# zz9tf/multimodal-fusion

Measured on AMD Instinct MI355X. Metric: similarity-pairs/sec (NxN cosine+top-k), higher is better.
Workload: dtype f16 MFMA scan + f32 exact re-rank; 1 GPU; N=262144 d=512 single-modality cosine + top-5, self excluded, f32 features, unit-norm Gaussian rows; rows_per_rank=262144, parallelism=single GPU, driver=single, scan_kernel=scan_b16x<f16> (v_mfma_f32_16x16x32_f16), col_splits=1, scan_grid=2048, fallback_rows=0, overflow_rows=0, query_order=False, near_duplicate_rows_estimate=0

## Files before the change

### multimodal-fusion_amd/csrc/mmf_api.hip

```cpp
#include <stdarg.h>
#include <string.h>

#include <algorithm>
#include <map>
#include <mutex>
#include <optional>
#include <utility>
#include <vector>

#include "mmf_host.h"

namespace mmf {

static thread_local char g_err[512] = "";

void set_error(const char* fmt, ...) {
  va_list ap;
  va_start(ap, fmt);
  vsnprintf(g_err, sizeof(g_err), fmt, ap);
  va_end(ap);
}

struct WsEntry { char* base = nullptr; size_t cap = 0; WsKept kept; };
static std::mutex g_ws_mu;
// ... 253 lines not shown
  int32_t* fail_rows = nullptr; uint32_t *fail_count = nullptr, *cand_total = nullptr;
  uint32_t h_fail4[4] = {0, 0, 0, 0};
  std::vector<uint32_t> h_tot;
  static size_t bytes(int64_t n) { return ws_bytes(n, 4) + ws_bytes(4, 4) + ws_bytes(256, 4); }
  void carve(Workspace& ws, int64_t n) { fail_rows = ws.take<int32_t>(n); fail_count = ws.take<uint32_t>(4); cand_total = ws.take<uint32_t>(256); }
  int zero(hipStream_t s) const {
    MMF_HIP(hipMemsetAsync(fail_count, 0, 16, s)); MMF_HIP(hipMemsetAsync(cand_total, 0, 1024, s));
    return MMF_OK;
  }
  int read(bool totals, hipStream_t s) {
    MMF_HIP(hipMemcpyAsync(h_fail4, fail_count, 16, hipMemcpyDeviceToHost, s));
    h_tot.assign(totals ? 256 : 0, 0);
    if (totals) MMF_HIP(hipMemcpyAsync(h_tot.data(), cand_total, 1024, hipMemcpyDeviceToHost, s));
    MMF_HIP(hipStreamSynchronize(s));
    return MMF_OK;
  }
};

static void symmetric_live_mode(bool* live, bool* forward) {
  const char* e = getenv("MMF_SYMMETRIC_LIVE");
  const int v = e ? atoi(e) : 1;
  *live = (v == 1 || v == 2);
  *forward = (v == 0 || v == 2);
}
static bool symmetric_prune_mode() {
  const char* e = getenv("MMF_SYMMETRIC_PRUNE");
  return !e || atoi(e) != 0;
}
static bool wide_sink_mode() {
  const char* e = getenv("MMF_WIDE_SINK");
  return !e || atoi(e) != 0;
}
static constexpr int64_t kSymMinRows = 131072;
static bool symmetric_scan_wanted(int64_t n, int dp, int bcap, int metric, int forced_splits, bool same_ids, int* G) {
  if (!same_ids || dp != 512 || bcap != scan_bf16_cap(1, 512) || forced_splits != 0) return false;
  if (metric != MMF_DOT && metric != MMF_COSINE) return false;
  const int64_t nb = (n + 255) / 256;
  if (nb * 256 * 1024 >= (int64_t(1) << 32)) return false;
  const char* e = getenv("MMF_SYMMETRIC");
  const int mode = e ? atoi(e) : -1;
  if (mode == 0 || (mode < 0 && n < kSymMinRows)) return false;
  int g = sym_default_group(nb);
  if (const char* ge = getenv("MMF_SYMMETRIC_G")) { const int v = atoi(ge); if (v >= 1 && v <= 65536) g = v; }
  *G = g;
  return true;
}
// ... 152 lines not shown
  int64_t n, m; int kk, cap, bcap, splits, lists, fb_splits; int64_t FB;
  CandLists L;
  ExactLists XL;
  FlagBlock flags;
  char* scan_scratch = nullptr;
  char* order_scratch = nullptr;
  int order_mode = MMF_QUERY_ORDER_OFF; bool order_try = false;
  char* qo_scratch = nullptr; uint16_t* qo_Z = nullptr; float *qo_zn = nullptr, *qo_rn = nullptr, *qo_un = nullptr;
  int64_t n_pad_q() const { return (n + 255) / 256 * 256; }
  int set_query_order(int mode) {
    if (mode < MMF_QUERY_ORDER_AUTO || mode > MMF_QUERY_ORDER_ON) { set_error("simtopk: bad query_order %d", mode); return MMF_E_INVALID; }
    order_mode = mode;
    order_try = !wide && (mode == MMF_QUERY_ORDER_ON || (mode == MMF_QUERY_ORDER_AUTO && n >= 32768 && m >= 32768));
    return MMF_OK;
  }

  bool sym_try = false; int sym_G = 32; int lists_alloc = 0;
  SymBuffers sym;
  WsKept sym_kept; WsKept* sym_keep = nullptr;
  uint32_t* sym_cnt = nullptr; uint2* sym_ent = nullptr;
  int64_t sym_grid() const { return sym_schedule_grid((n + 255) / 256, sym_G); }
  void set_symmetric(int G) {
    sym_try = true; sym_G = G;
    if (lists_alloc < 4) lists_alloc = 4;
  }
  CandLists view(bool symmetric) const {
    CandLists v = L;
    v.lists = symmetric ? 4 : lists;
    if (v.lists <= 2) { v.keys = nullptr; v.margin = nullptr; }
    v.spill_stacks = spill_stacks_for(v.lists);
    if (symmetric) { v.sym_cnt = sym_cnt; v.sym_ent = sym_ent; v.sym_cap = kSymCap; }
    return v;
  }

  int dp, panels;
  bool wide = false;
  int panel_splits[16]; int max_splits = 1;
  int64_t n_seed;
  int32_t* seed = nullptr;
  int64_t seed_stripes() const { return wide ? 3 : 2; }
  static constexpr int64_t kRowsExactMax = 48;
  int64_t rows_exact_cap = 0;
  float* row_keys = nullptr;
  bool leave_floors = false; int out_stride = 0;
  float* floor_key_out = nullptr; uint32_t* floor_id_out = nullptr;
  int64_t failed_rows = 0;
  FastTail(int64_t n_, int64_t m_, int kk_, int forced_splits, int dp_, int panels_ = 1, int64_t m_panel_min = -1,
           int64_t m_panel_max = -1)
      : n(n_), m(m_), kk(kk_), cap(scan_f32_cap(kk_)), dp(dp_), panels(panels_) {
    wide = dp > 1024;
    bcap = wide ? scan_b16w_cap(kk) : scan_bf16_cap(kk, dp);
// ... 78 lines not shown
      if (order_mode == MMF_QUERY_ORDER_ON || near_rows >= 8 * (int64_t)query_order_pivots()) {
        MMF_TRY(launch_query_order_apply(fo.q.Z, fo.q.zn, fo.q.rn, fo.q.un, n, n_pad_q(), fo.dp, fo.f16, qo_scratch, qo_Z, qo_zn, qo_rn, qo_un, &fo.perm, s));
        fo.q.Z = qo_Z; fo.q.zn = qo_zn; fo.q.rn = qo_rn; fo.q.un = qo_un;
      }
      MMF_TRY(t_order.stop(s));
    }
    const bool symmetric = sym_try && !fo.perm && fo.n_panels == 0;
    const CandLists L = view(symmetric);
    MMF_HIP(hipMemsetAsync(L.overflow, 0, (size_t)n * 4, s));
    MMF_TRY(flags.zero(s));
    EventTimer t_scan, t_sel, t_fb;
    EventTimer t_panel[16];
    int grid = 0;
    MMF_HIP(hipMemsetAsync(seed, 0x80, (size_t)n_seed * 4 * seed_stripes(), s));
    MMF_HIP(hipMemsetAsync(L.spill_cnt, 0, (size_t)n * 4, s));
    MMF_TRY(t_scan.start(profile, s));
    ScanB16Panel pn;
    pn.seed = seed; pn.seed_stride = n_seed;
    pn.share = (splits > 1 || fo.n_panels > 1) ? 1 : 0;
    ScanB16Problem sp(fo.q, fo.c, n, m, fo.m_pad_tiles, fo.dp, r.d, fo.f16, r.metric, kk);
    if (symmetric) {
      bool live, forward;
      symmetric_live_mode(&live, &forward);
      const WsKept tables{sym.sched, (n + 255) / 256, sym_G, forward ? 1 : 0};
      MMF_TRY(launch_scan_b16_sym(sp, SymLaunch{sym_G, live, forward, symmetric_prune_mode(), !(sym_kept == tables)}, L, scan_scratch, sym,
                                  pn, s, &grid));
      if (sym_keep) *sym_keep = tables;
    } else if (fo.n_panels == 0) {
      if (wide) {
        CandLists Lw = L;
        if (!wide_sink_mode()) { Lw.spill_cnt = nullptr; Lw.spill_ids = nullptr; Lw.spill_cap = 0; Lw.spill_stacks = 0; }
        pn.sunk = seed + 2 * n_seed;
        MMF_TRY(launch_scan_b16w(sp, splits, Lw, pn, s, &grid));
      }
      else MMF_TRY(launch_scan_b16(sp, splits, L, scan_scratch, pn, s, &grid));
    } else {
      int list_base = 0;
      for (int p = 0; p < fo.n_panels; ++p) {
        const mmf_panel& P = fo.panels[p];
        if (P.ready_event) MMF_HIP(hipStreamWaitEvent(s, static_cast<hipEvent_t>(P.ready_event), 0));
        MMF_TRY(t_panel[p].start(profile, s));
        pn.list_base = list_base;
        list_base += 2 * panel_splits[p];
        pn.seg_len = (uint32_t)P.seg_len; pn.seg_stride = (uint32_t)P.seg_stride; pn.id_off = (uint32_t)P.id_base;
        sp.ZC = P.Z; sp.cb = P.cb; sp.m = P.m; sp.m_pad = P.m_pad;
        MMF_TRY(launch_scan_b16(sp, panel_splits[p], L, scan_scratch, pn, s, &grid));
        MMF_TRY(t_panel[p].stop(s));
      }
    }
    MMF_TRY(launch_scan_b16_audit(pn, L.overflow, n, s));
    if (const char* e = getenv("MMF_DEBUG_FLAG_ROWS")) {
      const int64_t f = atoll(e);
      if (f > 0) MMF_HIP(hipMemsetAsync(L.overflow, 1, (size_t)(f < n ? f : n) * 4, s));
    }
    MMF_TRY(t_scan.stop(s));
    if (symmetric && getenv("MMF_SYMMETRIC_DEBUG")) {
      MMF_HIP(hipStreamSynchronize(s));
      std::vector<uint32_t> hc((size_t)n), hl((size_t)sym_grid() * 8);
      uint32_t none = 0;
      MMF_HIP(hipMemcpy(hc.data(), sym_cnt, hc.size() * 4, hipMemcpyDeviceToHost));
      MMF_HIP(hipMemcpy(hl.data(), sym.log_cnt, hl.size() * 4, hipMemcpyDeviceToHost));
      MMF_HIP(hipMemcpy(&none, sym.none_cnt, 4, hipMemcpyDeviceToHost));
      unsigned long long tot = 0, logged = 0; uint32_t mx = 0, lmx = 0;
      for (uint32_t v : hc) { tot += v; if (v > mx) mx = v; }
      for (uint32_t v : hl) { logged += v; if (v > lmx) lmx = v; }
      bool live, forward;
      symmetric_live_mode(&live, &forward);
      fprintf(stderr, "[mmf symmetric] G %d grid %lld %s %s: rows without a threshold %u, received entries %llu (%.1f per row, largest %u of %d), fullest wave log %u of %d, logged entries %llu (%.1f per row, filing %s)\n",
              sym_G, (long long)sym_grid(), live ? "live" : "frozen", forward ? "ahead" : "back", none, tot, (double)tot / (double)n, mx,
              kSymCap, lmx, kSymLogPerWave, logged, (double)logged / (double)n, symmetric_prune_mode() ? "pruned" : "complete");
    }
    if (select_wait_event) MMF_HIP(hipStreamWaitEvent(s, static_cast<hipEvent_t>(select_wait_event), 0));

    SelectProblem q = r.select();
    q.rx = fo.rx; q.cy = fo.cy; q.perm = fo.perm;
    q.fail_rows = flags.fail_rows; q.fail_count = flags.fail_count; q.cand_total = r.stats ? flags.cand_total : nullptr;
    q.two_pass = true;
    q.order_scratch = getenv("MMF_SELECT_UNORDERED") ? nullptr : order_scratch;
    q.out_stride = out_stride;
    if (leave_floors) { q.floor_key_out = floor_key_out; q.floor_id_out = floor_id_out; }
    MMF_TRY(t_sel.start(profile, s));
    MMF_TRY(launch_select(q, L, s));
    MMF_TRY(t_sel.stop(s));

    MMF_TRY(flags.read(r.stats != nullptr, s));
    const uint32_t* h_fail4 = flags.h_fail4;
    const uint32_t h_fail = h_fail4[0];
    failed_rows = h_fail;
    if (h_fail > 0 && getenv("MMF_DEBUG_PRINT_FLAGGED")) {
      const uint32_t nshow = h_fail < 8 ? h_fail : 8;
      int32_t rows[8];
      MMF_HIP(hipMemcpy(rows, flags.fail_rows, nshow * sizeof(int32_t), hipMemcpyDeviceToHost));
      for (uint32_t i = 0; i < nshow; ++i) {
// ... 650 lines not shown
  if (!one) { MMF_TRY(t[0].stop(s)); MMF_TRY(t[1].start(r.profile, s)); }
  std::vector<uint32_t> h_tot(stats ? 256 : 0);
  MMF_TRY(ex.run(ws, B, one ? t : nullptr, stats ? &h_tot : nullptr));
  if (!one) MMF_TRY(t[1].stop(s));
  fill_stats(stats, MMF_PREC_EXACT, ex.splits(ex.pieces[0]), ex.grid, t[0].ms(), t[1].ms(), t[2].ms(), 0.f, 0, 0, 0, h_tot);
  return MMF_OK;
}

}

using namespace mmf;

extern "C" {

int mmf_version(void) { return MMF_ABI_VERSION; }
int mmf_debug_query_order(int32_t* perm_host, int64_t n) { return query_order_last(perm_host, n); }
int64_t mmf_debug_symmetric_schedule(int64_t row_blocks, int group, int launch, int32_t* table_host, int64_t capacity) {
  if (row_blocks < 1 || group < 1 || launch < 0 || launch > 1) { set_error("debug_symmetric_schedule: bad argument"); return MMF_E_INVALID; }
  const int64_t grid = sym_schedule_grid(row_blocks, group);
  if (table_host) {
    if (capacity < grid) { set_error("debug_symmetric_schedule: table of %lld entries needed", (long long)grid); return MMF_E_INVALID; }
    bool live, forward;
    symmetric_live_mode(&live, &forward);
    sym_schedule_table(row_blocks, group, launch, table_host, forward);
  }
  return grid;
}
const char* mmf_last_error(void) { return g_err; }

int mmf_release_workspaces(void) {
  std::lock_guard<std::mutex> lk(g_ws_mu);
  query_order_forget();
  for (auto& slot : g_ws) {
    for (auto& kv : slot) {
      if (kv.second.base) {
        int prev = -1;
        (void)hipGetDevice(&prev);
        (void)hipSetDevice(kv.first.first);
        (void)hipDeviceSynchronize();
        (void)hipFree(kv.second.base);
        if (prev >= 0) (void)hipSetDevice(prev);
      }
    }
    slot.clear();
  }
  for (auto& kv : g_stage) {
    int prev = -1;
// ... 2825 lines not shown
```

### multimodal-fusion_amd/csrc/mmf_host.h

```cpp
#pragma once
#include <hip/hip_runtime.h>
#include <functional>
#include <optional>
#include <stdint.h>
#include <stdio.h>

#include <string>
#include <vector>

#include "../../include/mmf_hg.h"
#include "../../include/mmf_hg_topk.h"
#include "../../include/mmf_hg_topk16.h"
#include "../../include/ext/mmf_hg_topk16_seg.h"
#include "../../include/ext/mmf_hg_topk_xy.h"
#include "../../include/ext/mmf_hg_seg_exact.h"
#include "../../include/ext/mmf_hg_topk_anyk.h"
#include "../../include/ext/mmf_hg_kmeans_ragged.h"
#include "../../include/ext/mmf_hg_cross_seg.h"
#include "../../include/ext/mmf_hg_cross_seg16.h"
#include "../../include/ext/mmf_hg_cross_segw.h"
#include "../../include/ext/mmf_hg_fast_anyk.h"
#include "../../include/ext/mmf_hg_wide_anyk.h"
#include "../../include/ext/mmf_hg_seg_anyk.h"
#include "../../include/ext/mmf_hg_cross_seg_anyk.h"
// ... 11 lines not shown
      mmf::set_error("%s failed: %s (%s:%d)", #call, hipGetErrorString(_e), __FILE__, __LINE__); \
      return MMF_E_HIP;                                                                    \
    }                                                                                      \
  } while (0)

#define MMF_LAUNCH_CHECK()                                                                 \
  do {                                                                                     \
    hipError_t _e = hipGetLastError();                                                     \
    if (_e != hipSuccess) {                                                                \
      mmf::set_error("kernel launch failed: %s (%s:%d)", hipGetErrorString(_e), __FILE__, __LINE__); \
      return MMF_E_HIP;                                                                    \
    }                                                                                      \
  } while (0)

#define MMF_TRY(expr)            \
  do {                           \
    int _rc = (expr);            \
    if (_rc != MMF_OK) return _rc; \
  } while (0)

struct WsKept {
  const void* where = nullptr;
  int64_t row_blocks = 0;
  int group = 0, forward = 0;
  bool operator==(const WsKept& o) const { return where == o.where && row_blocks == o.row_blocks && group == o.group && forward == o.forward; }
};

struct Workspace {
  char* base = nullptr;
  size_t cap = 0;
  size_t off = 0;
  WsKept kept;
  WsKept* keep = nullptr;
  void reset() { off = 0; }
  template <typename T>
  T* take(size_t count) {
    size_t bytes = (count * sizeof(T) + 255) & ~size_t(255);
    T* p = reinterpret_cast<T*>(base + off);
    off += bytes;
    return p;
  }
};
inline size_t ws_bytes(size_t count, size_t elem) { return (count * elem + 255) & ~size_t(255); }

int upload_table(hipStream_t s, void* dst, const void* src_host, size_t bytes);

struct DeviceGuard {
  int prev = -1;
// ... 48 lines not shown


int launch_row_scalars(const void* X, int64_t n, int64_t d, int dtype, int metric, float* out,
                       uint32_t* max_n, hipStream_t s);

struct CandLists {
  uint32_t* cnt;
  uint32_t* ids;
  uint32_t* overflow;
  int lists;
  int cap;
  float* keys = nullptr;
  float* margin = nullptr;
  int slot_ulp = 16;
  uint32_t* spill_cnt = nullptr;
  uint32_t* spill_ids = nullptr;
  int spill_cap = 0;
  int spill_stacks = 0;
  uint32_t* sym_cnt = nullptr;
  uint2* sym_ent = nullptr;
  int sym_cap = 0;
};

int64_t sym_schedule_grid(int64_t nb, int G);
void sym_schedule_table(int64_t nb, int G, int launch, int32_t* out, bool forward = false);
int sym_default_group(int64_t nb);
constexpr int kSymCap = 512;
constexpr int kSymLogPerWave = 4096;
struct SymBuffers {
  float* thr = nullptr;
  uint32_t* log = nullptr;
  uint32_t* log_cnt = nullptr;
  int32_t* sched = nullptr;
  uint32_t* none_cnt = nullptr;
  static size_t bytes(int64_t n_pad, int64_t grid) {
    return ws_bytes(n_pad, 4) + ws_bytes((size_t)grid * 8 * kSymLogPerWave * 4, 4) + ws_bytes((size_t)grid * 8, 4) +
           ws_bytes((size_t)grid * 16, 4) + ws_bytes(4, 4);
  }
  void carve(Workspace& ws, int64_t n_pad, int64_t grid) {
    thr = ws.take<float>(n_pad); log = ws.take<uint32_t>((size_t)grid * 8 * kSymLogPerWave * 4);
    log_cnt = ws.take<uint32_t>((size_t)grid * 8); sched = ws.take<int32_t>((size_t)grid * 16); none_cnt = ws.take<uint32_t>(4);
  }
};

struct ScanB16Panel {
  int list_base = 0;
  uint32_t seg_len = 0, seg_stride = 0, id_off = 0;
  int32_t* seed = nullptr;
// ... 103 lines not shown
};
struct PrepRows { const void* X; int64_t n, d; int dtype, metric; const float* scal; const uint32_t* max_n; };
int launch_prep_half(const PrepRows& r, const HalfImage& out, int dp, bool f16, hipStream_t s);
int launch_prep_half_gather(const PrepRows& r, const int32_t* gather, int64_t n_pos, const HalfImage& out, int dp, bool f16, hipStream_t s);

struct ScanB16Problem {
  const void* ZQ; const float *q_zn, *q_rn, *q_un;
  const void* ZC; const float* cb; const uint32_t* maxima;
  int64_t n_rows, m, m_pad;
  int dp; int64_t d; bool f16; int metric, kk;
  ScanB16Problem(const HalfImage& q, const HalfImage& c, int64_t n_rows_, int64_t m_, int64_t m_pad_, int dp_, int64_t d_, bool f16_,
                 int metric_, int kk_)
      : ZQ(q.Z), q_zn(q.zn), q_rn(q.rn), q_un(q.un), ZC(c.Z), cb(c.cb), maxima(c.maxima), n_rows(n_rows_), m(m_), m_pad(m_pad_),
        dp(dp_), d(d_), f16(f16_), metric(metric_), kk(kk_) {}
};
int launch_scan_b16(const ScanB16Problem& p, int col_splits, const CandLists& L, void* scratch, const ScanB16Panel& pn, hipStream_t s,
                    int* grid_out);
int launch_scan_b16_audit(const ScanB16Panel& pn, uint32_t* overflow, int64_t n_rows, hipStream_t s);
int launch_scan_b16_ceil(const ScanB16Problem& p, int col_splits, const CandLists& L, void* scratch, const ScanB16Panel& pn, const float* ceil,
                         hipStream_t s, int* grid_out);
int launch_scan_b16_ceilings(const ScanB16Problem& p, int cap, const float* floor_key, const float* rx, const uint32_t* max_n, float lambda,
                             int64_t n_pad, float* ceil, hipStream_t s);
size_t scan_b16_sym_scratch_bytes(int64_t n_rows, int G);
struct SymLaunch { int G; bool live, forward, prune, tables; };
int launch_scan_b16_sym(const ScanB16Problem& p, const SymLaunch& y, const CandLists& L, void* scratch, const SymBuffers& sb,
                        const ScanB16Panel& pn, hipStream_t s, int* grid_out);
size_t scan_b16_scratch_bytes(int64_t n_rows, int col_splits, int dp, int cap);
int scan_bf16_slot_ulp(int cap);
int scan_b16_queries_per_block(int dp);
size_t scan_b16_seg_scratch_bytes(int64_t grid, int dp, int cap);
int launch_scan_b16_seg(const ScanB16Problem& p, const int32_t* sched, int64_t grid, const CandLists& L, void* scratch,
                        const ScanB16Panel& pn, hipStream_t s);
int launch_scan_b16_seg_ceil(const ScanB16Problem& p, const int32_t* sched, int64_t grid, const CandLists& L, void* scratch,
                             const ScanB16Panel& pn, const float* ceil, hipStream_t s);
int launch_scan_b16_ceilings_gather(const ScanB16Problem& p, int cap, const int32_t* gather, int64_t n_pos, const float* floor_key, const float* rx,
                                    const uint32_t* max_n, float lambda, int64_t nq_pad, float* ceil, hipStream_t s);
int launch_scan_b16_xseg(const ScanB16Problem& p, const int32_t* sched, int64_t grid, const uint32_t* bounds, const CandLists& L,
                         void* scratch, const ScanB16Panel& pn, hipStream_t s);
int launch_scan_b16_xseg_ceil(const ScanB16Problem& p, const int32_t* sched, int64_t grid, const uint32_t* bounds, const CandLists& L,
                              void* scratch, const ScanB16Panel& pn, const float* ceil, hipStream_t s);

struct AnykStage { const int64_t* idx; const float* val; const float* key; int64_t n; int depth; int64_t col_offset; };
int launch_anyk_count(const AnykStage& st, const int32_t* fail_rows, const uint32_t* fail_count, const float* floor_key, const uint32_t* floor_id,
                      int32_t* certified, uint32_t* hist, hipStream_t s);
int launch_anyk_emit(const AnykStage& st, const int32_t* certified, int t, int done, int out_stride, int64_t* out_idx, float* out_val,
                     float* floor_key, uint32_t* floor_id, int32_t* rescan_rows, uint32_t* rescan_count, hipStream_t s);
int launch_anyk_iota(int32_t* rows, int64_t n, hipStream_t s);
// ... 162 lines not shown
```

### multimodal-fusion_amd/csrc/mmf_scan_bf16.hip

```cpp
#include <stdlib.h>

#include <type_traits>

#include "mmf_dev.h"
#include "mmf_host.h"

namespace mmf {

constexpr int B_CT = 32;
#ifndef MMF_B_CAP
#define MMF_B_CAP 15
#endif
constexpr int B_CAP = MMF_B_CAP;
constexpr int B_CAP_BIG = 16;
constexpr int B_CAP_WIDE = 32;

typedef __bf16 bf16x8_t __attribute__((ext_vector_type(8)));
typedef _Float16 f16x8_t __attribute__((ext_vector_type(8)));
typedef uint32_t u32x4 __attribute__((ext_vector_type(4)));

struct PrepArgs {
  const void* X; int64_t n; int64_t d; int dtype; int metric;
  const float* scal;
  const uint32_t* max_n;
// ... 137 lines not shown
  int share;
  int kk;
  int metric;
  int d;
  int debug;
  unsigned long long* dbg;
  uint32_t* lids;
  uint32_t* cand_cnt; uint32_t* cand_ids; uint32_t* overflow;
  float* cand_keys;
  float* margin_out;
  uint32_t* spill_cnt; uint32_t* spill_ids; int spill_cap;
  int spill_stacks;
  const int32_t* sched;
  float* sym_thr;
  int sym_live;
  uint32_t* sym_log;
  uint32_t* sym_log_cnt;
  int sym_log_cap;
  const uint32_t* xbounds;
  const float* ceil;
};

enum { SEG_QPOS = 0, SEG_ROW0 = 1, SEG_NQ = 2, SEG_T0 = 3, SEG_T1 = 4, SEG_IDOFF = 5, SEG_ENTRY = 8 };
enum { SYM_RB = 0, SYM_B1 = 1, SYM_N1 = 2, SYM_B2 = 3, SYM_N2 = 4 };
enum { XSEG_SLOT = 5, XSEG_W0 = 6, XSEG_W1 = 7 };

__device__ __forceinline__ int32_t seed_enc(float f) {
  const int32_t b = __float_as_int(f);
  return b >= 0 ? b : (b ^ 0x7fffffff);
}
constexpr int32_t kSeedNone = (int32_t)0x80808080;

__device__ __forceinline__ float scan_margin(int metric, int d, int dp, int cap, float zn, float rn, float un, const uint32_t* maxima) {
  const float ZB = __uint_as_float(maxima[0]), RB = __uint_as_float(maxima[1]);
  const float UB = __uint_as_float(maxima[2]), CB = __uint_as_float(maxima[3]);
  const float g_acc = (float)(dp + 8) * 5.9604645e-8f;
  const float g_chain = (float)(d + 2) * 5.9604645e-8f;
  const float slot_eps = (cap <= 16) ? 1.9073486e-6f : 3.8146973e-6f;
  const float e1 = rn * ZB + un * RB + (g_acc + slot_eps) * (zn * ZB + CB);
  float e2;
  if (metric == MMF_DOT) e2 = g_chain * un * UB;
  else if (metric == MMF_COSINE) e2 = (g_chain + 4.7683716e-7f) * un * UB * 1.01f;
  else e2 = g_chain * un * UB + 2.3841858e-7f * (un * un + UB * UB);
  return 2.0f * (e1 + e2) * 1.001f + 1e-30f;
}

__device__ __forceinline__ void glds4(const void* gptr, const void* lptr) {
// ... 38 lines not shown

  const int tid = threadIdx.x;
  const int lane = tid & 63;
  const int wave = __builtin_amdgcn_readfirstlane(tid >> 6);
  const int khalf = SPLITK ? wave / NQW : 0;
  const int qw = SPLITK ? wave % NQW : wave;
  const bool owner = khalf == 0;
  const int half = lane >> 5;
  const int g = lane >> 4;
  const int c16 = lane & 15;
  const int ownb = g & 1;
  const int c = c16 + 16 * ownb;

  int64_t rb;
  int split;
  int64_t t_begin, t_end, row0 = 0;
  int nq = 0;
  uint32_t id_off = a.id_off;
  int sym_n1 = 0, sym_skip = 0;
  int xw0 = 0, xw1 = 0;
  if constexpr (SYM != 0) {
    const int32_t* e = a.sched + (size_t)blockIdx.x * SEG_ENTRY;
    if (e[SYM_RB] < 0) return;
    rb = e[SYM_RB]; split = 0;
    t_begin = e[SYM_B1]; t_end = t_begin + e[SYM_N1] + e[SYM_N2];
    sym_n1 = e[SYM_N1]; sym_skip = e[SYM_B2] - (e[SYM_B1] + e[SYM_N1]);
  } else if constexpr (SEG) {
    const int32_t* e = a.sched + (size_t)blockIdx.x * SEG_ENTRY;
    rb = e[SEG_QPOS] / QT; row0 = e[SEG_ROW0]; nq = e[SEG_NQ];
    t_begin = e[SEG_T0]; t_end = e[SEG_T1];
    if constexpr (XSEG) {
      id_off = 0u; split = e[XSEG_SLOT];
      xw0 = e[XSEG_W0] - e[SEG_T0]; xw1 = e[XSEG_W1] - e[SEG_T0];
    } else {
      id_off = (uint32_t)e[SEG_IDOFF];
      split = 0;
    }
  } else {
    const int CS = a.conc_splits;
    const int64_t round = blockIdx.x / a.blocks_per_round;
    const int64_t j = blockIdx.x - round * a.blocks_per_round;
    const int64_t q = j >> 3;
    const int x = (int)(j & 7);
    split = (int)round * CS + x % CS;
    rb = q * (8 / CS) + x / CS;
    if (rb >= a.row_blocks) return;
    t_begin = (int64_t)split * a.tiles_per_split;
// ... 208 lines not shown
        const uint32_t j0 = id_base + (uint32_t)tt * B_CT + 4u * (uint32_t)g;
#pragma unroll
        for (int cb = 0; cb < 2; ++cb) {
#pragma unroll
          for (int jj = 0; jj < 4; ++jj) {
            const uint32_t j = j0 + 16u * cb + jj;
            if ((uint32_t)(j - b0.x) < b0.y) x.t[cb][0][jj] = kNegInf;
            if ((uint32_t)(j - b1.x) < b1.y) x.t[cb][1][jj] = kNegInf;
          }
        }
      }
    }
  };
  float thr_q0, thr_q1;
  auto refresh_thr = [&]() {
    const float mine = list.thr;
    const float theirs = __shfl_xor(mine, 16);
    thr_q0 = ownb ? theirs : mine;
    thr_q1 = ownb ? mine : theirs;
  };
  refresh_thr();

  constexpr bool SYMCNT = SYM != 0 && MMF_SYM_COUNT != 0;
  auto filter = [&](const Acc& acc, int tt, float m0, float m1) {
    if (__builtin_expect(!(DBG && (a.debug & 1)) && !(SYM != 0 && (MMF_SYM_ABLATE_Q & SYM) != 0) && __any((m0 >= thr_q0) || (m1 >= thr_q1)), 0)) {
      uint32_t id0 = id_base + (uint32_t)tt * B_CT;
      if constexpr (SYM != 0) id0 += (tt >= sym_n1) ? (uint32_t)(sym_skip * B_CT) : 0u;
      f32x16 v;
#pragma unroll
      for (int cb = 0; cb < 2; ++cb) {
#pragma unroll
        for (int j = 0; j < 4; ++j) {
          const float mine = ownb ? acc.t[cb][1][j] : acc.t[cb][0][j];
          const float give = ownb ? acc.t[cb][0][j] : acc.t[cb][1][j];
          v[4 * cb + j] = mine;
          v[8 + 4 * cb + j] = __shfl_xor(give, 16);
        }
      }
      if constexpr (CEIL) {
        float ce;
        if constexpr (XSEG) {
          const int ln = (int)__builtin_amdgcn_mbcnt_hi(~0u, __builtin_amdgcn_mbcnt_lo(~0u, 0u));
          ce = (a.ceil + (q0 + 32 * qw))[(ln & 15) + (ln & 16)];
        } else ce = a.ceil[qop];
#pragma unroll
        for (int r = 0; r < 16; ++r) v[r] = (v[r] > ce) ? kNegInf : v[r];
      }
// ... 188 lines not shown
  if (a.spill_stacks && a.spill_cnt) {
    const uint32_t mine = qvalid ? list.sink.cpos : 0u;
    const uint32_t theirs = (uint32_t)__shfl_xor((int)mine, 32);
    if (mine + theirs > (uint32_t)a.spill_cap) list.lost = kFltMax;
    if (qvalid && half == 0 && (mine | theirs)) a.spill_cnt[qpos] = mine | (theirs << 16);
  }
  sync_seed();
  if constexpr (SYM == 2) {
    if (MMF_SYM_ABLATE == 3) sym_wcnt = 0;
    if (lane == 0) a.sym_log_cnt[(size_t)blockIdx.x * NW + wave] = sym_wcnt < (uint32_t)a.sym_log_cap ? sym_wcnt : (uint32_t)a.sym_log_cap;
  }
  if (qvalid) {
    const int64_t lbase = qpos * a.lists_total + a.list_base + 2 * split + half;
    a.cand_cnt[lbase] = (uint32_t)list.cnt;
    for (int e = 0; e < list.cnt; ++e) {
      uint32_t id = list.id_of(e);
      if (a.seg_len) id = (id / a.seg_len) * a.seg_stride + id % a.seg_len;
      a.cand_ids[lbase * CAP + e] = id + id_off;
      if (a.cand_keys) a.cand_keys[lbase * CAP + e] = list.keys[e * NTL];
    }
    if (a.cand_keys && half == 0) a.margin_out[qpos] = margin;
    if (list.lost > kNegInf) atomicMax(a.lost + qpos, seed_enc(list.lost) + SlotList<CAP, NTL>::SLOTS);
  }
}

__global__ void audit_kernel(const int32_t* seed, const int32_t* lost, uint32_t* overflow, int64_t n) {
  const int64_t i = (int64_t)blockIdx.x * blockDim.x + threadIdx.x;
  if (i >= n) return;
  const int32_t l = lost[i];
  if (l > kSeedNone && l >= seed[i]) overflow[i] = 1u;
}

struct CeilArgs {
  const float* floor_key; const float* rx;
  const float *q_zn, *q_rn, *q_un; const uint32_t* maxima; const uint32_t* max_n;
  int64_t n, n_pad; int metric, d, dp, cap; float lambda;
  float* ceil;
  const int32_t* gather;
};
template <bool GATHER>
__global__ void ceil_kernel(CeilArgs a) {
  const int64_t i = (int64_t)blockIdx.x * blockDim.x + threadIdx.x;
  if (i >= a.n_pad) return;
  if (i >= a.n) { a.ceil[i] = __builtin_huge_valf(); return; }
  int64_t row = i;
  if constexpr (GATHER) {
// ... 284 lines not shown
    return launch_b16_t<64, 8, 1, B_CAP, true, true, 0, true, true>(a, f16, grid, s);
  }
  set_error("scan_b16_xseg_ceil: no kernel for padded dim %d with %d-entry lists (full-depth passes only)", dp, cap);
  return MMF_E_INTERNAL;
}

int launch_scan_b16_xseg_ceil(const ScanB16Problem& p, const int32_t* sched, int64_t grid, const uint32_t* bounds, const CandLists& L,
                              void* scratch, const ScanB16Panel& pn, const float* ceil, hipStream_t s) {
  if (grid <= 0) return MMF_OK;
  if (L.lists < 2 || (L.lists & 1) || !bounds || !sched) { set_error("scan_b16_xseg_ceil: list pairs, a work table and the rows' bounds expected"); return MMF_E_INTERNAL; }
  if (L.lists > 2 && (!L.keys || !L.margin)) { set_error("scan_b16_xseg_ceil: several list pairs need keys and margins"); return MMF_E_INTERNAL; }
  if (!pn.seed) { set_error("scan_b16_xseg_ceil: threshold buffers missing"); return MMF_E_INTERNAL; }
  if (!ceil) { set_error("scan_b16_xseg_ceil: ceilings missing"); return MMF_E_INTERNAL; }
  ScanB16Args a = scan_args(p, L, pn, scratch);
  a.sched = sched; a.xbounds = bounds; a.share = pn.share; a.ceil = ceil;
  return launch_b16_xseg_ceil_for(p.dp, L.cap, a, p.f16, grid, s);
}

int sym_default_group(int64_t nb) {
  int64_t g = (nb + 31) / 32;
  return (int)(g < 32 ? 32 : g);
}
static int64_t sym_super_blocks(int64_t nb, int G) { const int64_t ns = nb / G; return ns < 1 ? 1 : ns; }
int64_t sym_schedule_grid(int64_t nb, int G) {
  const int64_t ns = sym_super_blocks(nb, G);
  return ((ns + 7) / 8 + (nb > ns * G ? 1 : 0)) * 8 * G;
}
void sym_schedule_table(int64_t nb, int G, int launch, int32_t* out, bool forward) {
  const int64_t ns = sym_super_blocks(nb, G), grid = sym_schedule_grid(nb, G), tiles = nb * 8;
  const int64_t per = 8 * (int64_t)G, stretches = (ns + 7) / 8;
  auto first_tile = [&](int64_t sb) { return sb * G * 8; };
  auto end_tile = [&](int64_t sb) { return sb == ns - 1 ? tiles : (sb + 1) * G * 8; };
  for (int64_t b = 0; b < grid; ++b) {
    int32_t* e = out + b * SEG_ENTRY;
    for (int i = 0; i < SEG_ENTRY; ++i) e[i] = 0;
    e[SYM_RB] = -1;
    int64_t sb = (b / per) * 8 + (b % 8), rbi = sb * G + (b % per) / 8;
    if (b / per >= stretches) {
      if (b % 8 != (ns - 1) % 8) continue;
      sb = ns - 1; rbi = ns * G + (b % per) / 8;
    } else if (sb >= ns) continue;
    if (rbi >= nb) continue;
    int64_t b1 = 0, n1 = 0, b2 = 0, n2 = 0;
    if (launch == 0) {
      b1 = first_tile(sb); n1 = end_tile(sb) - b1;
      if (ns >= 2 && (ns % 2) == 0) { const int64_t o = (sb + ns / 2) % ns; b2 = first_tile(o); n2 = end_tile(o) - b2; }
    } else {
      const int64_t h = (ns - 1) / 2;
      if (h == 0) continue;
      int64_t lo = forward ? sb + 1 : sb - h, hi = lo + h - 1;
      if (lo >= ns) { lo -= ns; hi -= ns; }
      if (lo < 0) { lo += ns; hi += ns; }
      if (hi < ns) { b1 = first_tile(lo); n1 = end_tile(hi) - b1; }
      else { b1 = first_tile(lo); n1 = end_tile(ns - 1) - b1; b2 = 0; n2 = end_tile(hi - ns); }
    }
    if (n2 == 0) b2 = b1 + n1;
    e[SYM_RB] = (int32_t)rbi; e[SYM_B1] = (int32_t)b1; e[SYM_N1] = (int32_t)n1; e[SYM_B2] = (int32_t)b2; e[SYM_N2] = (int32_t)n2;
  }
}

__global__ void sym_thr_kernel(const int32_t* seed, float* thr, int64_t n, int64_t n_pad, uint32_t* none_cnt) {
  const int64_t i = (int64_t)blockIdx.x * blockDim.x + threadIdx.x;
  if (i >= n_pad) return;
  if (i >= n) { thr[i] = __builtin_huge_valf(); return; }
  const int32_t o = seed[i];
  if (o > kSeedNone) { thr[i] = __int_as_float(o >= 0 ? o : (o ^ 0x7fffffff)); return; }
  thr[i] = -kFltMax;
  atomicAdd(none_cnt, 1u);
}

__global__ __launch_bounds__(256) void sym_scatter_kernel(const uint32_t* log, const uint32_t* log_cnt, int log_cap, uint32_t* sym_cnt,
                                                          uint2* sym_ent, int cap, int32_t* lost,
                                                          const int32_t* seed, int slot_ulp) {
  const uint32_t c = log_cnt[blockIdx.x];
  const u32x4* lg = reinterpret_cast<const u32x4*>(log) + (size_t)blockIdx.x * log_cap;
  for (uint32_t e = threadIdx.x; e < c; e += 256) {
    const u32x4 v = lg[e];
    if (seed) {
      const int32_t sd = seed[v[0]], b = (int32_t)v[2];
      if (sd > kSeedNone && (b >= 0 ? b : (b ^ 0x7fffffff)) + slot_ulp < sd) continue;
    }
    const uint32_t slot = atomicAdd(sym_cnt + v[0], 1u);
    if (slot < (uint32_t)cap) {
      sym_ent[(size_t)v[0] * cap + slot] = make_uint2(v[1], v[2]);
    } else {
      atomicMax(lost + v[0], 0x7fffffff);
    }
  }
}

size_t scan_b16_sym_scratch_bytes(int64_t n_rows, int G) {
  const int64_t nb = (n_rows + 255) / 256;
  return (size_t)sym_schedule_grid(nb, G) * 16 * 512 * 4 + 256;
}

int launch_scan_b16_sym(const ScanB16Problem& p, const SymLaunch& y, const CandLists& L, void* scratch, const SymBuffers& sb,
                        const ScanB16Panel& pn, hipStream_t s, int* grid_out) {
  const int64_t n = p.n_rows, nb = (n + 255) / 256, n_pad = nb * 256, grid = sym_schedule_grid(nb, y.G);
  if (p.metric != MMF_DOT && p.metric != MMF_COSINE) {
    set_error("scan_b16_sym: metric %d has a per-candidate bias, which the symmetric kernels do not apply", p.metric);
    return MMF_E_INTERNAL;
  }
  if (L.lists != 4 || L.cap != B_CAP || !L.keys || !L.margin || !L.sym_cnt || !pn.seed) { set_error("scan_b16_sym: lists missing"); return MMF_E_INTERNAL; }
  if (n_pad * 1024 >= (int64_t(1) << 32)) { set_error("scan_b16_sym: operand image beyond the 32-bit tile offsets"); return MMF_E_INTERNAL; }
  if (y.tables) {
    std::vector<int32_t> tab((size_t)grid * 2 * SEG_ENTRY);
    sym_schedule_table(nb, y.G, 0, tab.data(), y.forward);
    sym_schedule_table(nb, y.G, 1, tab.data() + (size_t)grid * SEG_ENTRY, y.forward);
    MMF_TRY(upload_table(s, sb.sched, tab.data(), tab.size() * 4));
  }
  MMF_HIP(hipMemsetAsync(L.sym_cnt, 0, (size_t)n * 4, s));
  MMF_HIP(hipMemsetAsync(L.cnt, 0, (size_t)n * L.lists * 4, s));
  MMF_HIP(hipMemsetAsync(sb.log_cnt, 0, (size_t)grid * 8 * 4, s));
  MMF_HIP(hipMemsetAsync(sb.none_cnt, 0, 16, s));
  ScanB16Args a = scan_args(p, L, pn, scratch);
  a.ZQ = p.ZC;
  a.tiles_total = n_pad / B_CT; a.row_blocks = nb;
  a.spill_stacks = 0;
  a.sched = sb.sched;
  a.sym_thr = sb.thr; a.sym_live = y.live ? 1 : 0; a.sym_log = sb.log; a.sym_log_cnt = sb.log_cnt; a.sym_log_cap = kSymLogPerWave;
#if MMF_SYM_COUNT
  static unsigned long long* dbuf = nullptr;
  if (!dbuf) MMF_HIP(hipMalloc(&dbuf, 128));
  a.dbg = dbuf;
  auto report = [&](int launch) -> int {
    unsigned long long h[8];
    MMF_HIP(hipMemcpyAsync(h, dbuf, 64, hipMemcpyDeviceToHost, s));
    MMF_HIP(hipStreamSynchronize(s));
    fprintf(stderr, "[mmf sym count] launch %d: wave-tiles=%llu visits=%llu (cold %llu) hits=%llu entry-compactions=%llu lanes-with-hit=%llu\n",
            launch, h[5], h[0], h[1], h[2], h[3], h[4]);
    return MMF_OK;
// ... 24 lines not shown
```

Baseline: 2090 billion pairs/s.

## Split symmetric scan second launch into two phases with antipodal pairing

Restructures the symmetric scan schedule so the second launch runs in two phases. Phase A covers the backward half-window without wraparound, and phase B covers the wrapped tail, writing to a third list-pair slot. An optional antipodal mode moves the opposite super-block pairing from the first launch into the second. The aim is to balance work across workgroups and cut wasted wraparound tiles, at the cost of a larger grid, an extra candidate list pair (more memory and memsets) and a more complex schedule table.

```diff
diff --git a/multimodal-fusion_amd/csrc/mmf_api.hip b/multimodal-fusion_amd/csrc/mmf_api.hip
--- a/multimodal-fusion_amd/csrc/mmf_api.hip
+++ b/multimodal-fusion_amd/csrc/mmf_api.hip
@@ -299,6 +299,14 @@
   const int v = e ? atoi(e) : 1;
   *live = (v == 1 || v == 2);
   *forward = (v == 0 || v == 2);
+}
+static constexpr int kSymAntipodalMinGroup = 32;
+static void symmetric_schedule_mode(int* phases, bool* antipodal, int G, int schedule_default = 2) {
+  const char* e = getenv("MMF_SYMMETRIC_PHASES");
+  const int v = e ? atoi(e) : schedule_default;
+  *phases = v == 1 ? 1 : (v == 2 ? 2 : schedule_default);
+  const char* a = getenv("MMF_SYMMETRIC_ANTIPODAL");
+  *antipodal = a ? atoi(a) == 1 : (*phases == 2 && G >= kSymAntipodalMinGroup);
 }
 static bool symmetric_prune_mode() {
   const char* e = getenv("MMF_SYMMETRIC_PRUNE");
@@ -497,11 +505,11 @@
   int64_t sym_grid() const { return sym_schedule_grid((n + 255) / 256, sym_G); }
   void set_symmetric(int G) {
     sym_try = true; sym_G = G;
-    if (lists_alloc < 4) lists_alloc = 4;
+    if (lists_alloc < 2 * kSymListPairs) lists_alloc = 2 * kSymListPairs;
   }
   CandLists view(bool symmetric) const {
     CandLists v = L;
-    v.lists = symmetric ? 4 : lists;
+    v.lists = symmetric ? 2 * kSymListPairs : lists;
     if (v.lists <= 2) { v.keys = nullptr; v.margin = nullptr; }
     v.spill_stacks = spill_stacks_for(v.lists);
     if (symmetric) { v.sym_cnt = sym_cnt; v.sym_ent = sym_ent; v.sym_cap = kSymCap; }
@@ -626,9 +634,11 @@
     if (symmetric) {
       bool live, forward;
       symmetric_live_mode(&live, &forward);
-      const WsKept tables{sym.sched, (n + 255) / 256, sym_G, forward ? 1 : 0};
-      MMF_TRY(launch_scan_b16_sym(sp, SymLaunch{sym_G, live, forward, symmetric_prune_mode(), !(sym_kept == tables)}, L, scan_scratch, sym,
-                                  pn, s, &grid));
+      int phases; bool antipodal;
+      symmetric_schedule_mode(&phases, &antipodal, sym_G);
+      const WsKept tables{sym.sched, (n + 255) / 256, sym_G, forward ? 1 : 0, phases, antipodal ? 1 : 0};
+      MMF_TRY(launch_scan_b16_sym(sp, SymLaunch{sym_G, live, forward, symmetric_prune_mode(), !(sym_kept == tables), phases, antipodal}, L,
+                                  scan_scratch, sym, pn, s, &grid));
       if (sym_keep) *sym_keep = tables;
     } else if (fo.n_panels == 0) {
       if (wide) {
@@ -670,9 +680,15 @@
       for (uint32_t v : hl) { logged += v; if (v > lmx) lmx = v; }
       bool live, forward;
       symmetric_live_mode(&live, &forward);
-      fprintf(stderr, "[mmf symmetric] G %d grid %lld %s %s: rows without a threshold %u, received entries %llu (%.1f per row, largest %u of %d), fullest wave log %u of %d, logged entries %llu (%.1f per row, filing %s)\n",
+      int phases; bool antipodal;
+      symmetric_schedule_mode(&phases, &antipodal, sym_G);
+      const size_t first_b = (size_t)sym_schedule_phase_b_begin((n + 255) / 256, sym_G) * 8;
+      unsigned long long logged_b = 0;
+      for (size_t i = first_b; i < hl.size(); ++i) logged_b += hl[i];
+      fprintf(stderr, "[mmf symmetric] G %d grid %lld %s %s: rows without a threshold %u, received entries %llu (%.1f per row, largest %u of %d), fullest wave log %u of %d, logged entries %llu (%.1f per row, filing %s), phases %d antipodal %d, logged by phase B %llu (%.1f per row)\n",
               sym_G, (long long)sym_grid(), live ? "live" : "frozen", forward ? "ahead" : "back", none, tot, (double)tot / (double)n, mx,
-              kSymCap, lmx, kSymLogPerWave, logged, (double)logged / (double)n, symmetric_prune_mode() ? "pruned" : "complete");
+              kSymCap, lmx, kSymLogPerWave, logged, (double)logged / (double)n, symmetric_prune_mode() ? "pruned" : "complete",
+              forward ? 1 : phases, (antipodal && !forward) ? 1 : 0, logged_b, (double)logged_b / (double)n);
     }
     if (select_wait_event) MMF_HIP(hipStreamWaitEvent(s, static_cast<hipEvent_t>(select_wait_event), 0));
 
@@ -1369,7 +1385,9 @@
     if (capacity < grid) { set_error("debug_symmetric_schedule: table of %lld entries needed", (long long)grid); return MMF_E_INVALID; }
     bool live, forward;
     symmetric_live_mode(&live, &forward);
-    sym_schedule_table(row_blocks, group, launch, table_host, forward);
+    int phases; bool antipodal;
+    symmetric_schedule_mode(&phases, &antipodal, group, 1);
+    sym_schedule_table(row_blocks, group, launch, table_host, forward, phases, antipodal);
   }
   return grid;
 }
diff --git a/multimodal-fusion_amd/csrc/mmf_host.h b/multimodal-fusion_amd/csrc/mmf_host.h
--- a/multimodal-fusion_amd/csrc/mmf_host.h
+++ b/multimodal-fusion_amd/csrc/mmf_host.h
@@ -57,8 +57,11 @@
 struct WsKept {
   const void* where = nullptr;
   int64_t row_blocks = 0;
-  int group = 0, forward = 0;
-  bool operator==(const WsKept& o) const { return where == o.where && row_blocks == o.row_blocks && group == o.group && forward == o.forward; }
+  int group = 0, forward = 0, phases = 0, antipodal = 0;
+  bool operator==(const WsKept& o) const {
+    return where == o.where && row_blocks == o.row_blocks && group == o.group && forward == o.forward && phases == o.phases &&
+           antipodal == o.antipodal;
+  }
 };
 
 struct Workspace {
@@ -153,8 +156,10 @@
   int sym_cap = 0;
 };
 
+constexpr int kSymListPairs = 3;
 int64_t sym_schedule_grid(int64_t nb, int G);
-void sym_schedule_table(int64_t nb, int G, int launch, int32_t* out, bool forward = false);
+int64_t sym_schedule_phase_b_begin(int64_t nb, int G);
+void sym_schedule_table(int64_t nb, int G, int launch, int32_t* out, bool forward = false, int phases = 1, bool antipodal = false);
 int sym_default_group(int64_t nb);
 constexpr int kSymCap = 512;
 constexpr int kSymLogPerWave = 4096;
@@ -304,7 +309,7 @@
 int launch_scan_b16_ceilings(const ScanB16Problem& p, int cap, const float* floor_key, const float* rx, const uint32_t* max_n, float lambda,
                              int64_t n_pad, float* ceil, hipStream_t s);
 size_t scan_b16_sym_scratch_bytes(int64_t n_rows, int G);
-struct SymLaunch { int G; bool live, forward, prune, tables; };
+struct SymLaunch { int G; bool live, forward, prune, tables; int phases = 2; bool antipodal = false; };
 int launch_scan_b16_sym(const ScanB16Problem& p, const SymLaunch& y, const CandLists& L, void* scratch, const SymBuffers& sb,
                         const ScanB16Panel& pn, hipStream_t s, int* grid_out);
 size_t scan_b16_scratch_bytes(int64_t n_rows, int col_splits, int dp, int cap);
diff --git a/multimodal-fusion_amd/csrc/mmf_scan_bf16.hip b/multimodal-fusion_amd/csrc/mmf_scan_bf16.hip
--- a/multimodal-fusion_amd/csrc/mmf_scan_bf16.hip
+++ b/multimodal-fusion_amd/csrc/mmf_scan_bf16.hip
@@ -183,7 +183,7 @@
 };
 
 enum { SEG_QPOS = 0, SEG_ROW0 = 1, SEG_NQ = 2, SEG_T0 = 3, SEG_T1 = 4, SEG_IDOFF = 5, SEG_ENTRY = 8 };
-enum { SYM_RB = 0, SYM_B1 = 1, SYM_N1 = 2, SYM_B2 = 3, SYM_N2 = 4 };
+enum { SYM_RB = 0, SYM_B1 = 1, SYM_N1 = 2, SYM_B2 = 3, SYM_N2 = 4, SYM_SLOT = 5, SYM_PHASE = 6 };
 enum { XSEG_SLOT = 5, XSEG_W0 = 6, XSEG_W1 = 7 };
 
 __device__ __forceinline__ int32_t seed_enc(float f) {
@@ -268,7 +268,7 @@
   if constexpr (SYM != 0) {
     const int32_t* e = a.sched + (size_t)blockIdx.x * SEG_ENTRY;
     if (e[SYM_RB] < 0) return;
-    rb = e[SYM_RB]; split = 0;
+    rb = e[SYM_RB]; split = SYM == 2 ? e[SYM_SLOT] : 0;
     t_begin = e[SYM_B1]; t_end = t_begin + e[SYM_N1] + e[SYM_N2];
     sym_n1 = e[SYM_N1]; sym_skip = e[SYM_B2] - (e[SYM_B1] + e[SYM_N1]);
   } else if constexpr (SEG) {
@@ -523,7 +523,9 @@
   refresh_thr();
 
   constexpr bool SYMCNT = SYM != 0 && MMF_SYM_COUNT != 0;
+  float ablate_keep = -kFltMax;
   auto filter = [&](const Acc& acc, int tt, float m0, float m1) {
+    if (SYM != 0 && (MMF_SYM_ABLATE_Q & SYM) != 0 && (MMF_SYM_ABLATE_Q & 4) != 0) ablate_keep = fmaxf(ablate_keep, fmaxf(m0, m1));
     if (__builtin_expect(!(DBG && (a.debug & 1)) && !(SYM != 0 && (MMF_SYM_ABLATE_Q & SYM) != 0) && __any((m0 >= thr_q0) || (m1 >= thr_q1)), 0)) {
       uint32_t id0 = id_base + (uint32_t)tt * B_CT;
       if constexpr (SYM != 0) id0 += (tt >= sym_n1) ? (uint32_t)(sym_skip * B_CT) : 0u;
@@ -758,6 +760,7 @@
     if (a.cand_keys && half == 0) a.margin_out[qpos] = margin;
     if (list.lost > kNegInf) atomicMax(a.lost + qpos, seed_enc(list.lost) + SlotList<CAP, NTL>::SLOTS);
   }
+  if (SYM != 0 && (MMF_SYM_ABLATE_Q & SYM) != 0 && (MMF_SYM_ABLATE_Q & 4) != 0) lids[tid & (NTL - 1)] = __float_as_uint(ablate_keep);
 }
 
 __global__ void audit_kernel(const int32_t* seed, const int32_t* lost, uint32_t* overflow, int64_t n) {
@@ -1088,40 +1091,70 @@
   return (int)(g < 32 ? 32 : g);
 }
 static int64_t sym_super_blocks(int64_t nb, int G) { const int64_t ns = nb / G; return ns < 1 ? 1 : ns; }
-int64_t sym_schedule_grid(int64_t nb, int G) {
+static int64_t sym_phase_a_grid(int64_t nb, int G) {
   const int64_t ns = sym_super_blocks(nb, G);
   return ((ns + 7) / 8 + (nb > ns * G ? 1 : 0)) * 8 * G;
 }
-void sym_schedule_table(int64_t nb, int G, int launch, int32_t* out, bool forward) {
-  const int64_t ns = sym_super_blocks(nb, G), grid = sym_schedule_grid(nb, G), tiles = nb * 8;
+int64_t sym_schedule_phase_b_begin(int64_t nb, int G) { return sym_phase_a_grid(nb, G); }
+int64_t sym_schedule_grid(int64_t nb, int G) {
+  const int64_t ns = sym_super_blocks(nb, G), h = (ns - 1) / 2;
+  if (h == 0) return sym_phase_a_grid(nb, G);
+  const int64_t pad = (ns % 8 == 0 && nb == ns * G) ? 8 : 0;
+  return sym_phase_a_grid(nb, G) + (h + 7) / 8 * 8 * G + pad;
+}
+void sym_schedule_table(int64_t nb, int G, int launch, int32_t* out, bool forward, int phases, bool antipodal) {
+  const int64_t ns = sym_super_blocks(nb, G), grid = sym_schedule_grid(nb, G), grid_a = sym_phase_a_grid(nb, G), tiles = nb * 8;
   const int64_t per = 8 * (int64_t)G, stretches = (ns + 7) / 8;
+  const int64_t h = (ns - 1) / 2;
+  if (forward) { phases = 1; antipodal = false; }
+  if (ns < 4 || (ns % 2) != 0) antipodal = false;
   auto first_tile = [&](int64_t sb) { return sb * G * 8; };
   auto end_tile = [&](int64_t sb) { return sb == ns - 1 ? tiles : (sb + 1) * G * 8; };
   for (int64_t b = 0; b < grid; ++b) {
     int32_t* e = out + b * SEG_ENTRY;
     for (int i = 0; i < SEG_ENTRY; ++i) e[i] = 0;
     e[SYM_RB] = -1;
-    int64_t sb = (b / per) * 8 + (b % 8), rbi = sb * G + (b % per) / 8;
-    if (b / per >= stretches) {
-      if (b % 8 != (ns - 1) % 8) continue;
-      sb = ns - 1; rbi = ns * G + (b % per) / 8;
+    const bool phase_b = b >= grid_a;
+    if (phase_b && (launch == 0 || phases != 2)) continue;
+    const int64_t bb = phase_b ? b - grid_a : b;
+    int64_t sb = (bb / per) * 8 + (bb % 8), rbi = sb * G + (bb % per) / 8;
+    if (phase_b) {
+      if (sb >= h) continue;
+    } else if (bb / per >= stretches) {
+      if (bb % 8 != (ns - 1) % 8) continue;
+      sb = ns - 1; rbi = ns * G + (bb % per) / 8;
     } else if (sb >= ns) continue;
     if (rbi >= nb) continue;
     int64_t b1 = 0, n1 = 0, b2 = 0, n2 = 0;
     if (launch == 0) {
       b1 = first_tile(sb); n1 = end_tile(sb) - b1;
-      if (ns >= 2 && (ns % 2) == 0) { const int64_t o = (sb + ns / 2) % ns; b2 = first_tile(o); n2 = end_tile(o) - b2; }
+      if (ns >= 2 && (ns % 2) == 0 && !antipodal) { const int64_t o = (sb + ns / 2) % ns; b2 = first_tile(o); n2 = end_tile(o) - b2; }
+    } else if (phase_b) {
+      b1 = first_tile(sb + ns - h); n1 = tiles - b1;
     } else {
-      const int64_t h = (ns - 1) / 2;
-      if (h == 0) continue;
-      int64_t lo = forward ? sb + 1 : sb - h, hi = lo + h - 1;
-      if (lo >= ns) { lo -= ns; hi -= ns; }
-      if (lo < 0) { lo += ns; hi += ns; }
-      if (hi < ns) { b1 = first_tile(lo); n1 = end_tile(hi) - b1; }
-      else { b1 = first_tile(lo); n1 = end_tile(ns - 1) - b1; b2 = 0; n2 = end_tile(hi - ns); }
+      const bool anti = antipodal && sb >= ns / 2;
+      if (h == 0 && !anti) continue;
+      if (h > 0) {
+        int64_t lo = forward ? sb + 1 : sb - h, hi = lo + h - 1;
+        if (phases == 2) { if (lo < 0) lo = 0; }
+        else {
+          if (lo >= ns) { lo -= ns; hi -= ns; }
+          if (lo < 0) { lo += ns; hi += ns; }
+        }
+        if (hi < lo) continue;
+        if (hi < ns) { b1 = first_tile(lo); n1 = end_tile(hi) - b1; }
+        else { b1 = first_tile(lo); n1 = end_tile(ns - 1) - b1; b2 = 0; n2 = end_tile(hi - ns); }
+      }
+      if (anti) {
+        const int64_t o = sb - ns / 2;
+        if (n1 == 0) { b1 = first_tile(o); n1 = end_tile(o) - b1; }
+        else { b2 = first_tile(o); n2 = end_tile(o) - b2; }
+      }
     }
     if (n2 == 0) b2 = b1 + n1;
     e[SYM_RB] = (int32_t)rbi; e[SYM_B1] = (int32_t)b1; e[SYM_N1] = (int32_t)n1; e[SYM_B2] = (int32_t)b2; e[SYM_N2] = (int32_t)n2;
+    e[SYM_SLOT] = phase_b ? 1 : 0;
+    e[SYM_PHASE] = launch == 0 || phases != 2 ? 0 : (phase_b ? 2 : 1);
   }
 }
 
@@ -1167,12 +1200,12 @@
     set_error("scan_b16_sym: metric %d has a per-candidate bias, which the symmetric kernels do not apply", p.metric);
     return MMF_E_INTERNAL;
   }
-  if (L.lists != 4 || L.cap != B_CAP || !L.keys || !L.margin || !L.sym_cnt || !pn.seed) { set_error("scan_b16_sym: lists missing"); return MMF_E_INTERNAL; }
+  if (L.lists != 2 * kSymListPairs || L.cap != B_CAP || !L.keys || !L.margin || !L.sym_cnt || !pn.seed) { set_error("scan_b16_sym: lists missing"); return MMF_E_INTERNAL; }
   if (n_pad * 1024 >= (int64_t(1) << 32)) { set_error("scan_b16_sym: operand image beyond the 32-bit tile offsets"); return MMF_E_INTERNAL; }
   if (y.tables) {
     std::vector<int32_t> tab((size_t)grid * 2 * SEG_ENTRY);
-    sym_schedule_table(nb, y.G, 0, tab.data(), y.forward);
-    sym_schedule_table(nb, y.G, 1, tab.data() + (size_t)grid * SEG_ENTRY, y.forward);
+    sym_schedule_table(nb, y.G, 0, tab.data(), y.forward, y.phases, y.antipodal);
+    sym_schedule_table(nb, y.G, 1, tab.data() + (size_t)grid * SEG_ENTRY, y.forward, y.phases, y.antipodal);
     MMF_TRY(upload_table(s, sb.sched, tab.data(), tab.size() * 4));
   }
   MMF_HIP(hipMemsetAsync(L.sym_cnt, 0, (size_t)n * 4, s));
```

Result: faster. 2116 billion pairs/s (median of 6 runs) (+1.3%).
